# Samleo8/RadarSLAMPy

Hardware: AMD Instinct MI355X
Metric: radar scan-pairs/sec (400x3768 polar) (higher is better)
Workload: dtype u8/f32/f64

## Files before the change

include/roam_abi.h:

```cpp
#ifndef ROAM_ABI_H
#define ROAM_ABI_H
#include <stdint.h>

#ifdef __cplusplus
extern "C" {
#endif

typedef struct roam_ctx roam_ctx;

enum {
    ROAM_OK = 0,
    ROAM_E_ARG = -1,
    ROAM_E_HIP = -2,
    ROAM_E_CAPACITY = -3,
    ROAM_E_NODEVICE = -4,
    ROAM_E_STATE = -5
};

#define ROAM_MAX_FEATURES 1024
#define ROAM_MAX_COLS 4096
#define ROAM_PYR_LEVELS 4

int32_t roam_create(int32_t device_id, roam_ctx **out);
int32_t roam_destroy(roam_ctx *ctx);
// ... 30 lines not shown
                               float *cart_f32, uint8_t *cart_u8);
int32_t roam_polar_to_cart_record_u8(roam_ctx *ctx, const uint8_t *rec, int32_t rows, int64_t stride,
                                     int32_t payload_off, int32_t clip, float *cart_f32,
                                     uint8_t *cart_u8);

#define ROAM_WARP_POLAR_LOG     1
#define ROAM_WARP_POLAR_INVERSE 2
int32_t roam_warp_polar_f32(roam_ctx *ctx, const float *src, int32_t n, int32_t rows, int32_t cols, int64_t src_row_stride,
                            int64_t src_image_stride, float *dst, int32_t dw, int32_t dh, float cx, float cy,
                            double max_radius, int32_t flags);

int32_t roam_klt_track_u8(roam_ctx *ctx, const uint8_t *prev_img, const uint8_t *next_img,
                          int32_t w, int32_t h, const float *pts, int32_t K,
                          float *next_pts, uint8_t *status, float *err);
int32_t roam_klt_track_f32(roam_ctx *ctx, const float *prev_img, const float *next_img,
                           int32_t w, int32_t h, const float *pts, int32_t K,
                           float *next_pts, uint8_t *status, float *err);
int32_t roam_pyr_down_u8(roam_ctx *ctx, const uint8_t *src, int32_t w, int32_t h, uint8_t *dst);

int32_t roam_reject_outliers(roam_ctx *ctx, const float *prev, const float *next, int32_t K,
                             double thr_px, int64_t node_limit, uint8_t *mask_out,
                             int32_t *n_inliers, int32_t *flags_out, uint64_t *adj_out);

int32_t roam_time_reject_outliers(roam_ctx *ctx, const float *prev, const float *next, int32_t K, int32_t copies,
                                  double thr_px, int64_t node_limit, int32_t reps, float *graph_ms, float *clique_ms,
                                  int32_t *n_inliers, int32_t *proven);

int32_t roam_kabsch2d(roam_ctx *ctx, const double *src, const double *tgt, int32_t N,
                      double *R, double *h);

int32_t roam_mds_solve(roam_ctx *ctx, const double *T_wj0, const double *p_w, const double *p_jt,
                       int32_t N, const double *T_wj_init, const double *sigma5, double period,
                       double *out6, int32_t *nfev, int32_t *info, double *x0_out, double *r0_out);
int32_t roam_mds_undistort(roam_ctx *ctx, const double *v3, const double *pts, int32_t N,
                           double period, double *out_xy, double *dT_out);

int32_t roam_ssc(roam_ctx *ctx, const double *kp, int32_t B, int32_t num_ret, double tol,
                 int32_t cols, int32_t rows, int32_t *sel_out, int32_t *n_sel);

int32_t roam_doh_maxima(roam_ctx *ctx, const float *img, int32_t w, int32_t h, const double *sigmas,
                        int32_t num_sigma, double threshold, int32_t *out_rcs, double *out_val,
                        int32_t cap, int32_t *n_out);

int32_t roam_log_maxima(roam_ctx *ctx, const void *img, int32_t img_bytes_per_px, int32_t w, int32_t h, int32_t num_sigma,
                        const int32_t *radius, const double *kernels, const double *scale, double threshold, int32_t *out_rcs,
                        double *out_val, int32_t cap, int32_t *n_out, double *out_layers);

int32_t roam_prune_blobs(const double *blobs, int32_t n, double overlap, uint8_t *keep_out);
int32_t roam_argsort_np122(const double *keys, int32_t n, int32_t *order_out);

int32_t roam_fmt_rotation(roam_ctx *ctx, const float *src_polar, const float *tgt_polar, int32_t rows, int32_t cols,
                          int32_t clip_px, int32_t downsample, double *angle_rad, double *scale, double *response);

int32_t roam_phase_correlate_f32(roam_ctx *ctx, const float *src, const float *tgt, int32_t batch, int32_t rows, int32_t cols,
                                 int64_t row_stride, int64_t image_stride, int32_t hanning, double *out_dxdy, double *out_response);

typedef struct roam_engine_cfg {
    int32_t lanes;
    int32_t rows;
    int32_t stride;
    int32_t payload_off;
    int32_t clip;
    int32_t pool_scans;
    int32_t peaks_cap;
    int32_t reject_outliers;
    int32_t motion_distortion;
// ... 105 lines not shown
```

radarslampy_amd/_ffi.py:

```python
import ctypes as C
import os
import threading

import numpy as np

_HERE = os.path.dirname(os.path.abspath(__file__))
LIB_PATH = os.environ.get("ROAM_LIB") or os.path.join(_HERE, "csrc", "libroam_hip.so")

ROAM_OK, ROAM_E_ARG, ROAM_E_HIP, ROAM_E_CAPACITY, ROAM_E_NODEVICE, ROAM_E_STATE = 0, -1, -2, -3, -4, -5
WARP_POLAR_LOG, WARP_POLAR_INVERSE = 1, 2
TIME_FFT_FIVE, TIME_DFT_FIVE, TIME_FFT_ROWS, TIME_FFT_TRANSPOSE, TIME_FFT_COLS = range(5)
PHASE_CORRELATE_MAX = 4096
MAX_FEATURES = 1024
STEP_NEW_SEQUENCE = 0x40000000


class RoamError(RuntimeError):
    def __init__(self, code, msg):
        super().__init__(f"libroam_hip error {code}: {msg}")
        self.code = code


class EngineCfg(C.Structure):
    _fields_ = [("lanes", C.c_int32), ("rows", C.c_int32), ("stride", C.c_int32), ("payload_off", C.c_int32),
# ... 21 lines not shown
_SIGS = {
    "roam_create": (C.c_int32, [C.c_int32, _P(_vp)]),
    "roam_destroy": (C.c_int32, [_vp]),
    "roam_last_error": (C.c_char_p, [_vp]),
    "roam_version": (C.c_char_p, []),
    "roam_device_info": (C.c_int32, [_vp, C.c_char_p, C.c_int32, _P(C.c_int32), _P(C.c_int64), C.c_char_p, C.c_int32]),
    "roam_synchronize": (C.c_int32, [_vp]),
    "roam_host_alloc": (C.c_int32, [_vp, C.c_int64, _P(_vp)]),
    "roam_host_free": (C.c_int32, [_vp, _vp]),
    "roam_png_decode_gray8": (C.c_int32, [_vp, C.c_int64, _vp, C.c_int64, C.c_int64, _P(C.c_int32), _P(C.c_int32)]),
    "roam_png_decode_file": (C.c_int32, [C.c_char_p, _vp, C.c_int64, C.c_int64, _P(C.c_int32), _P(C.c_int32)]),
    "roam_png_pool_create": (C.c_int32, [C.c_int32, _P(_vp)]),
    "roam_png_pool_submit": (C.c_int32, [_vp, C.c_char_p, _vp, C.c_int64, C.c_int64, C.c_int64]),
    "roam_png_pool_wait": (C.c_int32, [_vp, C.c_int64, _P(C.c_int32), _P(C.c_int32)]),
    "roam_png_pool_destroy": (C.c_int32, [_vp]),
    "roam_peaks_polar_f32": (C.c_int32, [_vp, _vp, C.c_int32, C.c_int32, _vp, C.c_int64, _P(C.c_int64)]),
    "roam_peaks_record_u8": (C.c_int32, [_vp, _vp, C.c_int32, C.c_int64, C.c_int32, C.c_int32, _vp, C.c_int64, _P(C.c_int64)]),
    "roam_peaks_polar_f32_cond": (C.c_int32, [_vp, _vp, C.c_int32, C.c_int32, C.c_double, C.c_double, C.c_double, _vp, C.c_int64,
                                              _P(C.c_int64)]),
    "roam_peaks_record_u8_cond": (C.c_int32, [_vp, _vp, C.c_int32, C.c_int64, C.c_int32, C.c_int32, C.c_double, C.c_double, C.c_double,
                                              _vp, C.c_int64, _P(C.c_int64)]),
    "roam_polar_to_cart_f32": (C.c_int32, [_vp, _vp, C.c_int32, C.c_int32, _vp, _vp]),
    "roam_polar_to_cart_record_u8": (C.c_int32, [_vp, _vp, C.c_int32, C.c_int64, C.c_int32, C.c_int32, _vp, _vp]),
    "roam_warp_polar_f32": (C.c_int32, [_vp, _vp, C.c_int32, C.c_int32, C.c_int32, C.c_int64, C.c_int64, _vp, C.c_int32, C.c_int32,
                                        C.c_float, C.c_float, C.c_double, C.c_int32]),
    "roam_klt_track_u8": (C.c_int32, [_vp, _vp, _vp, C.c_int32, C.c_int32, _vp, C.c_int32, _vp, _vp, _vp]),
    "roam_klt_track_f32": (C.c_int32, [_vp, _vp, _vp, C.c_int32, C.c_int32, _vp, C.c_int32, _vp, _vp, _vp]),
    "roam_pyr_down_u8": (C.c_int32, [_vp, _vp, C.c_int32, C.c_int32, _vp]),
    "roam_reject_outliers": (C.c_int32, [_vp, _vp, _vp, C.c_int32, C.c_double, C.c_int64, _vp, _P(C.c_int32), _P(C.c_int32), _vp]),
    "roam_time_reject_outliers": (C.c_int32, [_vp, _vp, _vp, C.c_int32, C.c_int32, C.c_double, C.c_int64, C.c_int32, _P(C.c_float), _P(C.c_float),
                                               _P(C.c_int32), _P(C.c_int32)]),
    "roam_kabsch2d": (C.c_int32, [_vp, _vp, _vp, C.c_int32, _vp, _vp]),
    "roam_mds_solve": (C.c_int32, [_vp, _vp, _vp, _vp, C.c_int32, _vp, _vp, C.c_double, _vp, _P(C.c_int32), _P(C.c_int32), _vp, _vp]),
    "roam_mds_undistort": (C.c_int32, [_vp, _vp, _vp, C.c_int32, C.c_double, _vp, _vp]),
    "roam_ssc": (C.c_int32, [_vp, _vp, C.c_int32, C.c_int32, C.c_double, C.c_int32, C.c_int32, _vp, _P(C.c_int32)]),
    "roam_doh_maxima": (C.c_int32, [_vp, _vp, C.c_int32, C.c_int32, _vp, C.c_int32, C.c_double, _vp, _vp, C.c_int32, _P(C.c_int32)]),
    "roam_log_maxima": (C.c_int32, [_vp, _vp, C.c_int32, C.c_int32, C.c_int32, C.c_int32, _vp, _vp, _vp, C.c_double, _vp, _vp, C.c_int32,
                                    _P(C.c_int32), _vp]),
    "roam_engine_create": (C.c_int32, [_vp, _P(EngineCfg)]),
    "roam_engine_destroy": (C.c_int32, [_vp]),
    "roam_engine_upload_scan": (C.c_int32, [_vp, C.c_int32, _vp]),
    "roam_engine_upload_scans_async": (C.c_int32, [_vp, C.c_int32, C.c_int32, _vp, C.c_int64]),
    "roam_engine_fence": (C.c_int32, [_vp]),
    "roam_engine_copy_scan": (C.c_int32, [_vp, C.c_int32, C.c_int32]),
    "roam_engine_init_lane": (C.c_int32, [_vp, C.c_int32, C.c_int32, _vp, C.c_int32, _vp]),
    "roam_engine_step": (C.c_int32, [_vp, _vp]),
    "roam_engine_results": (C.c_int32, [_vp, _P(LaneResult), C.c_int32]),
    "roam_engine_step_results": (C.c_int32, [_vp, C.c_int64, _P(LaneResult), C.c_int32]),
    "roam_engine_steps_enqueued": (C.c_int32, [_vp, _P(C.c_int64)]),
    "roam_engine_set_retrack": (C.c_int32, [_vp, C.c_int32]),
    "roam_engine_init_lane_detect": (C.c_int32, [_vp, C.c_int32, C.c_int32, _vp]),
    "roam_engine_init_lanes_detect": (C.c_int32, [_vp, C.c_int32, C.c_int32, _vp, _vp]),
    "roam_engine_lane_features": (C.c_int32, [_vp, C.c_int32, _vp, C.c_int32, _P(C.c_int32)]),
    "roam_engine_lane_peaks": (C.c_int32, [_vp, C.c_int32, _vp, C.c_int64, _P(C.c_int64)]),
    "roam_engine_doh_maxima": (C.c_int32, [_vp, C.c_int32, _vp, C.c_int32, C.c_double, _vp, _vp, C.c_int32, _P(C.c_int32)]),
    "roam_engine_lane_image": (C.c_int32, [_vp, C.c_int32, C.c_int32, _vp, C.c_int64]),
    "roam_engine_set_features": (C.c_int32, [_vp, C.c_int32, _vp, C.c_int32]),
    "roam_engine_kernel_avg": (C.c_int32, [_vp, C.c_char_p, C.c_int32, _P(C.c_float), _P(C.c_int32)]),
    "roam_engine_kernel_chunk_ms": (C.c_int32, [_vp, C.c_char_p, C.c_int32, _P(C.c_float), C.c_int32, _P(C.c_int32), _P(C.c_int32)]),
    "roam_engine_detect_chunk": (C.c_int32, [_vp, _P(C.c_int32)]),
    "roam_engine_map_reserve": (C.c_int32, [_vp, C.c_int32]),
    "roam_engine_map_count": (C.c_int32, [_vp, C.c_int32, _P(C.c_int32)]),
    "roam_engine_map_get": (C.c_int32, [_vp, C.c_int32, C.c_int32, _vp, _vp, _vp, C.c_int32, _P(C.c_int32), _P(C.c_int32)]),
    "roam_engine_stage_times": (C.c_int32, [_vp, _vp, _P(C.c_char_p), C.c_int32, _P(C.c_int32)]),
    "roam_engine_set_stage_events": (C.c_int32, [_vp, C.c_int32]),
    "roam_engine_time_kernel": (C.c_int32, [_vp, C.c_char_p, C.c_int32, _P(C.c_float), _P(C.c_double)]),
# ... 228 lines not shown
        return mask.astype(bool), n_in.value, flags.value, adj

    def time_reject_outliers(self, prev, new, thr_px, copies=4096, reps=3, node_limit=0):
        p = np.ascontiguousarray(prev, np.float32).reshape(-1, 2)
        n = np.ascontiguousarray(new, np.float32).reshape(-1, 2)
        g, q, ni, pr = C.c_float(0), C.c_float(0), C.c_int32(0), C.c_int32(0)
        self.check(self.lib.roam_time_reject_outliers(self.h, _ptr(p), _ptr(n), p.shape[0], int(copies), float(thr_px), int(node_limit), int(reps),
                                                      C.byref(g), C.byref(q), C.byref(ni), C.byref(pr)))
        return float(g.value), float(q.value), ni.value, bool(pr.value)

    def kabsch2d(self, src, tgt):
        s = np.ascontiguousarray(src, np.float64).reshape(-1, 2)
        t = np.ascontiguousarray(tgt, np.float64).reshape(-1, 2)
        R = np.empty((2, 2), np.float64)
        h = np.empty((2, 1), np.float64)
        self.check(self.lib.roam_kabsch2d(self.h, _ptr(s), _ptr(t), s.shape[0], _ptr(R), _ptr(h)))
        return R, h

    def mds_solve(self, T_wj0, p_w, p_jt, T_init, sigma5, period=0.25, want_debug=False):
        T0 = np.ascontiguousarray(T_wj0, np.float64)
        Ti = np.ascontiguousarray(T_init, np.float64)
        pw = np.ascontiguousarray(p_w[:, :2], np.float64)
        pj = np.ascontiguousarray(p_jt[:, :2], np.float64)
        sg = np.ascontiguousarray(sigma5, np.float64)
        N = pw.shape[0]
        out = np.empty(6)
        nfev, info = C.c_int32(0), C.c_int32(0)
        x0 = np.empty(6) if want_debug else None
        r0 = np.empty(2 * N + 3) if want_debug else None
        self.check(self.lib.roam_mds_solve(self.h, _ptr(T0), _ptr(pw), _ptr(pj), N, _ptr(Ti), _ptr(sg), float(period),
                                           _ptr(out), C.byref(nfev), C.byref(info), _ptr(x0), _ptr(r0)))
        return out, nfev.value, info.value, x0, r0

    def mds_undistort(self, v, pts, period=0.25):
        v = np.ascontiguousarray(v, np.float64)
        p = np.ascontiguousarray(pts[:, :2], np.float64)
        N = p.shape[0]
        xy = np.empty((N, 2))
        dT = np.empty(N)
        self.check(self.lib.roam_mds_undistort(self.h, _ptr(v), _ptr(p), N, float(period), _ptr(xy), _ptr(dT)))
        return xy, dT

    def ssc(self, kp, num_ret, tol, cols, rows):
        kp = np.ascontiguousarray(kp, np.float64)
        B = kp.shape[0]
        sel = np.empty(max(B, 1), np.int32)
        n = C.c_int32(0)
        self.check(self.lib.roam_ssc(self.h, _ptr(kp), B, int(num_ret), float(tol), int(cols), int(rows), _ptr(sel), C.byref(n)))
        return sel[:n.value]

    def fmt_rotation(self, src_polar, tgt_polar, clip_px=1012, downsample=10):
        a = np.ascontiguousarray(src_polar, np.float32)
        b = np.ascontiguousarray(tgt_polar, np.float32)
        assert a.shape == b.shape, "Images need to have the same shape!"
        ang, sc, rs = C.c_double(0), C.c_double(0), C.c_double(0)
        self.check(self.lib.roam_fmt_rotation(self.h, _ptr(a), _ptr(b), a.shape[0], a.shape[1], int(clip_px), int(downsample),
                                              C.byref(ang), C.byref(sc), C.byref(rs)))
        return ang.value, sc.value, rs.value

    def phase_correlate(self, src, tgt, hanning=True):
        a, b = phase_correlate_args(src, tgt)
        a, b = _f32_rows_in_place(a), _f32_rows_in_place(b)
        batch = a.ndim == 3
        a3, b3 = (a, b) if batch else (a[None], b[None])
        n, rows, cols = a3.shape
        if a3.strides[0 if n > 1 else 1:] != b3.strides[0 if n > 1 else 1:]:
# ... 74 lines not shown
```

radarslampy_amd/csrc/api.hip:

```cpp
#include "roam_internal.h"
#include <cmath>
#include <cstdlib>
#include <new>

extern "C" {

const char *roam_version(void) { return "radarslampy_amd 0.1 (gfx950, HIP)"; }

int32_t roam_create(int32_t device_id, roam_ctx **out)
{
    if (!out) return ROAM_E_ARG;
    *out = nullptr;
    int ndev = 0;
    if (hipGetDeviceCount(&ndev) != hipSuccess || ndev <= 0) return ROAM_E_NODEVICE;
    if (device_id < 0 || device_id >= ndev) return ROAM_E_ARG;
    roam_ctx *ctx = new (std::nothrow) roam_ctx();
    if (!ctx) return ROAM_E_HIP;
    ctx->device = device_id;
    if (hipSetDevice(device_id) != hipSuccess) { delete ctx; return ROAM_E_HIP; }
    hipDeviceProp_t prop;
    if (hipGetDeviceProperties(&prop, device_id) != hipSuccess) { delete ctx; return ROAM_E_HIP; }
    ctx->cu_count = prop.multiProcessorCount;
    if (hipStreamCreateWithFlags(&ctx->stream, hipStreamNonBlocking) != hipSuccess) { delete ctx; return ROAM_E_HIP; }
    if (hipStreamCreateWithFlags(&ctx->stream2, hipStreamNonBlocking) != hipSuccess) { hipStreamDestroy(ctx->stream); delete ctx; return ROAM_E_HIP; }
// ... 400 lines not shown
    ARG_CHECK(ctx, T_wj0 && p_w && p_jt && T_wj_init && sigma5 && out6 && N >= 2 && N <= 8 * ROAM_MAX_FEATURES && period > 0);
    const size_t m = 2 * (size_t)N + 3;
    SCRATCH(dT, double, S_IN0, sizeof(double) * 18);
    SCRATCH(dpw, double, S_IN1, sizeof(double) * 2 * (size_t)N);
    SCRATCH(dpj, double, S_IN2, sizeof(double) * 2 * (size_t)N);
    SCRATCH(dwork, double, S_TMP0, sizeof(double) * (m * 9 + N));
    SCRATCH(dout, double, S_OUT0, sizeof(double) * (6 + 6));
    SCRATCH(dr0, double, S_OUT1, sizeof(double) * m);
    SCRATCH(dint, int32_t, S_OUT2, sizeof(int32_t) * 2);
    double Tb[18];
    memcpy(Tb, T_wj0, sizeof(double) * 9);
    memcpy(Tb + 9, T_wj_init, sizeof(double) * 9);
    H2D(dT, Tb, sizeof(Tb));
    H2D(dpw, p_w, sizeof(double) * 2 * (size_t)N);
    H2D(dpj, p_jt, sizeof(double) * 2 * (size_t)N);
    MdsProblemDesc P;
    P.T_wj0 = dT; P.T_init = dT + 9; P.p_w = dpw; P.p_jt = dpj; P.count = nullptr;
    P.N = N; P.nstride = N; P.nmax = N; P.B = 1; P.period = period;
    for (int i = 0; i < 5; i++) P.sigma5[i] = sigma5[i];
    HIP_TRY(ctx, launch_mds_solve(ctx->stream, P, dwork, dout, dint, dint + 1, dout + 6, dr0));
    double o[12];
    int32_t ii[2];
    D2H(o, dout, sizeof(o));
    D2H(ii, dint, sizeof(ii));
    if (r0_out) D2H(r0_out, dr0, sizeof(double) * m);
    SYNC();
    memcpy(out6, o, sizeof(double) * 6);
    if (x0_out) memcpy(x0_out, o + 6, sizeof(double) * 6);
    if (nfev) *nfev = ii[0];
    if (info) *info = ii[1];
    return ROAM_OK;
}

extern "C" int32_t roam_mds_undistort(roam_ctx *ctx, const double *v3, const double *pts, int32_t N,
                                      double period, double *out_xy, double *dT_out)
{
    ENTER();
    ARG_CHECK(ctx, v3 && pts && N >= 0 && (out_xy || dT_out));
    if (N == 0) return ROAM_OK;
    SCRATCH(dv, double, S_IN0, sizeof(double) * 3);
    SCRATCH(dp, double, S_IN1, sizeof(double) * 2 * (size_t)N);
    SCRATCH(dxy, double, S_OUT0, sizeof(double) * 2 * (size_t)N);
    SCRATCH(ddt, double, S_OUT1, sizeof(double) * (size_t)N);
    H2D(dv, v3, sizeof(double) * 3);
    H2D(dp, pts, sizeof(double) * 2 * (size_t)N);
    HIP_TRY(ctx, launch_mds_undistort(ctx->stream, dv, dp, N, period, dxy, ddt));
    if (out_xy) D2H(out_xy, dxy, sizeof(double) * 2 * (size_t)N);
    if (dT_out) D2H(dT_out, ddt, sizeof(double) * (size_t)N);
    SYNC();
    return ROAM_OK;
}
```

radarslampy_amd/csrc/engine.hip:

```cpp
#include "roam_internal.h"
#include "retrack.h"
#include "kabsch_body.inc"
#include <algorithm>
#include <new>

#define KS ROAM_MAX_FEATURES
#define CART_CENTER 1012.0
#define M_PER_PX 0.0864
#define N_RETRACK 60
#define ROT_THR 0.2
#define TRANS_THR_SQ 4.0
#define ERR_THR 10.0f
#define TWO_PI 6.283185307179586476925286766559

#define RES_RING 8
enum { ST_PEAKS = 0, ST_WARP, ST_PYR, ST_KLT, ST_GRAPH, ST_CLIQUE, ST_KABSCH, ST_LM, ST_GLUE, ST_RETRACK, ST_COUNT };
static const char *kStageNames[ST_COUNT] = {"ingest_peaks", "warp_quantise", "pyramid", "klt", "consistency_graph",
                                            "max_clique", "kabsch", "mds_lm", "glue", "retrack"};

struct Engine {
    roam_engine_cfg cfg;
    int B = 0, W = 0, stage_cap = 0;
    PyrDesc pd;
    size_t rec_bytes = 0;
// ... 575 lines not shown
    ok = ok && dalloc(ctx, e, &e->feat, (size_t)B * KS * 2);
    ok = ok && dalloc(ctx, e, &e->feat_n, (size_t)B);
    ok = ok && dalloc(ctx, e, &e->klt_next, (size_t)B * KS * 2);
    ok = ok && dalloc(ctx, e, &e->klt_err, (size_t)B * KS);
    ok = ok && dalloc(ctx, e, &e->klt_status, (size_t)B * KS);
    ok = ok && dalloc(ctx, e, &e->good_old, (size_t)B * KS * 2);
    ok = ok && dalloc(ctx, e, &e->good_new, (size_t)B * KS * 2);
    ok = ok && dalloc(ctx, e, &e->good_idx, (size_t)B * KS);
    ok = ok && dalloc(ctx, e, &e->good_n, (size_t)B);
    ok = ok && dalloc(ctx, e, &e->adj, (size_t)B * KS * nw);
    ok = ok && dalloc(ctx, e, &e->cq_stack, (size_t)B * (KS + 2) * 2 * nw);
    ok = ok && dalloc(ctx, e, &e->cq_order, (size_t)B);
    ok = ok && dalloc(ctx, e, &e->cq_mask, (size_t)B * KS);
    ok = ok && dalloc(ctx, e, &e->cq_n, (size_t)B);
    ok = ok && dalloc(ctx, e, &e->cq_flags, (size_t)B);
    ok = ok && dalloc(ctx, e, &e->kab_src, (size_t)B * KS * 2);
    ok = ok && dalloc(ctx, e, &e->kab_tgt, (size_t)B * KS * 2);
    ok = ok && dalloc(ctx, e, &e->kab_out, (size_t)B * 6);
    ok = ok && dalloc(ctx, e, &e->in_n, (size_t)B);
    ok = ok && dalloc(ctx, e, &e->kf_pose, (size_t)B * 3);
    ok = ok && dalloc(ctx, e, &e->kf_vel, (size_t)B * 3) && dalloc(ctx, e, &e->kf_scan, (size_t)B) && dalloc(ctx, e, &e->kf_fresh, (size_t)B) &&
         dalloc(ctx, e, &e->kf_live, (size_t)B) && dalloc(ctx, e, &e->map_n, (size_t)B);
    ok = ok && dalloc(ctx, e, &e->kf_und, (size_t)B * KS * 2);
    ok = ok && dalloc(ctx, e, &e->kf_und_tmp, (size_t)B * KS * 2);
    ok = ok && dalloc(ctx, e, &e->pose, (size_t)B * 3);
    ok = ok && dalloc(ctx, e, &e->vel, (size_t)B * 3);
    ok = ok && dalloc(ctx, e, &e->T_wj0, (size_t)B * 9);
    ok = ok && dalloc(ctx, e, &e->T_init, (size_t)B * 9);
    ok = ok && dalloc(ctx, e, &e->p_w, (size_t)B * KS * 2);
    ok = ok && dalloc(ctx, e, &e->p_jt, (size_t)B * KS * 2);
    ok = ok && dalloc(ctx, e, &e->lm_work, (size_t)B * ((size_t)(2 * KS + 3) * 9 + KS));
    ok = ok && dalloc(ctx, e, &e->lm_out, (size_t)B * 6);
    ok = ok && dalloc(ctx, e, &e->lm_nfev, (size_t)B);
    ok = ok && dalloc(ctx, e, &e->lm_big, (size_t)2 * (1 + B));
    ok = ok && dalloc(ctx, e, &e->lm_info, (size_t)B);
    ok = ok && dalloc(ctx, e, &e->results, (size_t)B * RES_RING);
    if (ok && hipHostMalloc(reinterpret_cast<void **>(&e->results_host), sizeof(roam_lane_result) * (size_t)B * RES_RING, hipHostMallocDefault) != hipSuccess) {
        ROAM_SET_ERR(ctx, "engine: hipHostMalloc failed"); ok = false;
    }
    { const char *se = getenv("ROAM_STAGE_EVENTS"); e->stage_ev = !(se && se[0] == '0'); e->stage_ev_forced = se && (se[0] == '0' || se[0] == '1'); }
    e->rt_on = cfg->retrack_on_device != 0;
    if (ok && e->rt_on) {
        RtArgs &r = e->rt;
        memset(&r, 0, sizeof(r));
        const double step = (10.0 - 0.01) / 2.0;
        r.sigma1 = 1.0 * step + 0.01; r.sigma2 = 10.0; r.threshold = 0.0005;
        r.size1 = (int)(3 * r.sigma1); r.size2 = (int)(3 * r.sigma2);
        r.W = e->W; r.rows = cfg->rows; r.cols = cfg->clip; r.stride = cfg->stride; r.payload_off = cfg->payload_off;
        r.rec_bytes = (int64_t)e->rec_bytes;
        const int R = r.slots = std::max(1, std::min(B, cfg->retrack_slots > 0 ? cfg->retrack_slots : 2048));
        const size_t npx = (size_t)e->W * e->W;
        if (e->W > 2048) { ROAM_SET_ERR(ctx, "engine: device retrack needs a Cartesian image of at most 2048 x 2048"); roam_engine_destroy(ctx); return ROAM_E_ARG; }
        ok = ok && dalloc(ctx, e, &r.rt_n, 2) && dalloc(ctx, e, &r.rt_lane, (size_t)B) && dalloc(ctx, e, &r.rt_scan, (size_t)B);
        r.SP = (e->W + 15) & ~15;
        ok = ok && dalloc(ctx, e, &r.S, (size_t)r.SP * e->W * R);
        ok = ok && dalloc(ctx, e, const_cast<uint32_t **>(&r.boxtab), retrack_boxtab_words(e->W));
        ok = ok && dalloc(ctx, e, const_cast<uint32_t **>(&r.darktab), retrack_darktab_words(e->W));
        ok = ok && dalloc(ctx, e, const_cast<uint32_t **>(&r.phlist), retrack_phase_words(e->W));
        ok = ok && dalloc(ctx, e, &r.colT, (size_t)std::min(R, RT_TWO_PASS_SLOTS) * ((e->W + 63) / 64) * e->W);
        ok = ok && dalloc(ctx, e, &r.col_done, (size_t)std::min(R, RT_TWO_PASS_SLOTS) * 64);
        {
            const char *fv = getenv("ROAM_FUSED_DETECT");
            r.fused = (fv && fv[0] == '1') ? 1 : 0;
            e->det_side.chunk = getenv("ROAM_DET_SIDE") ? atoi(getenv("ROAM_DET_SIDE")) : ((B >= 2048 && r.slots >= 2048) ? 1024 : 0);
            r.fd_halo_words = (int64_t)retrack_fused_halo_words(e->W);
        }
        const size_t D = (size_t)B;
// ... 930 lines not shown
```

radarslampy_amd/csrc/kabsch_mds.hip:

```cpp
#include "roam_internal.h"

#define EPSMCH 2.220446049250313e-16
#define DWARF 2.2250738585072014e-308
#define LM_TMAX 256
#define TWO_PI 6.283185307179586476925286766559

#include "kabsch_body.inc"

__global__ __launch_bounds__(256) void kabsch_kernel(const double *__restrict__ src, const double *__restrict__ tgt,
                                                     const int32_t *__restrict__ count, int N, int nstride,
                                                     double *__restrict__ out6)
{
    __shared__ double red[8];
    const int b = blockIdx.x;
    kabsch_body(src + (int64_t)b * nstride * 2, tgt + (int64_t)b * nstride * 2, count ? count[b] : N, red, out6 + (int64_t)b * 6);
}

hipError_t launch_kabsch(hipStream_t st, const double *src, const double *tgt, const int32_t *count,
                         int N, int nstride, int B, double *out6)
{
    if (B <= 0) return hipSuccess;
    hipLaunchKernelGGL(kabsch_kernel, dim3(B), dim3(256), 0, st, src, tgt, count, N, nstride, out6);
    return hipGetLastError();
}
// ... 499 lines not shown
                    if (S.gnorm <= EPSMCH) info = 8;
                }
                S.info = info;
                S.ratio = ratio;
            }
            __syncthreads();
            if (S.accept) for (int i = t; i < m; i += (int)blockDim.x) fvec[i] = wa4[i];
            const int info = S.info;
            const double ratio = S.ratio;
            __syncthreads();
            LM_TICK(5)
            if (info != 0 || !(ratio < 1e-4)) break;
        }
        if (S.info != 0) break;
    }
#ifdef LM_TIMING
    if (x0_out && t == 0) for (int k = 0; k < 6; k++) x0_out[(size_t)b * 6 + k] = (double)tk[k];
#endif
    if (t < 6) out6[(size_t)b * 6 + t] = S.x[t];
    if (t == 0) { nfev_out[b] = S.nfev; info_out[b] = S.info; }
}

__global__ __launch_bounds__(LM_TMAX, LM_WPE) void mds_lm_kernel(MdsProblemDesc P, double *__restrict__ work_g,
                                                      double *__restrict__ out6, int32_t *__restrict__ nfev_out,
                                                      int32_t *__restrict__ info_out, double *__restrict__ x0_out,
                                                      double *__restrict__ r0_out, int lds_bytes, int wave_rows)
{
    extern __shared__ __align__(16) unsigned char lm_smem[];
    __shared__ LmShared S;
    if (!P.big || wave_rows == 0) {
        mds_lm_block_solve(P, blockIdx.x, work_g, out6, nfev_out, info_out, x0_out, r0_out, lds_bytes, wave_rows, lm_smem, S);
        return;
    }
    const int32_t *L = P.big + (size_t)P.big_slot * (1 + P.B);
    const int nbig = L[0];
    for (int q = blockIdx.x; q < nbig; q += (int)gridDim.x) {
        mds_lm_block_solve(P, L[1 + q], work_g, out6, nfev_out, info_out, x0_out, r0_out, lds_bytes, wave_rows, lm_smem, S);
        __syncthreads();
    }
    if (blockIdx.x == 0 && threadIdx.x == 0) P.big[(size_t)(P.big_slot ^ 1) * (1 + P.B)] = 0;
}

hipError_t launch_mds_solve(hipStream_t st, const MdsProblemDesc &p, double *work, double *out6,
                            int32_t *nfev, int32_t *info, double *x0_out, double *r0_out)
{
    if (p.B <= 0) return hipSuccess;
    const int ppt = std::min(4, (p.nmax + 2 + 63) / 64);
    const int wave_rows = 64 * ppt;
#define LMW_LAUNCH(PPT_) hipLaunchKernelGGL((mds_lm_wave_kernel<PPT_>), dim3(p.B), dim3(64), 0, st, p, out6, nfev, info, x0_out, r0_out)
    switch (ppt) {
    case 1: LMW_LAUNCH(1); break;
    case 2: LMW_LAUNCH(2); break;
    case 3: LMW_LAUNCH(3); break;
    default: LMW_LAUNCH(4); break;
    }
#undef LMW_LAUNCH
    hipError_t e = hipGetLastError();
    if (e != hipSuccess || p.nmax + 2 <= wave_rows) return e;
    const size_t mmax = 2 * (size_t)p.nmax + 3;
    size_t need = (mmax * 9 + p.nmax) * sizeof(double);
    const size_t cap = 32768;
    size_t lds = need <= cap ? need : cap;
    const int threads = p.nmax <= 448 ? 128 : LM_TMAX;
    const int grid = p.big ? std::min(p.B, 512) : p.B;
    hipLaunchKernelGGL(mds_lm_kernel, dim3(grid), dim3(threads), lds, st, p, work, out6, nfev, info, x0_out, r0_out, (int)lds, wave_rows);
    return hipGetLastError();
}

__global__ __launch_bounds__(256) void mds_undistort_kernel(const double *__restrict__ v3, const double *__restrict__ pts,
                                                            int N, double period, double *__restrict__ out_xy,
                                                            double *__restrict__ dT_out)
{
    const int i = blockIdx.x * 256 + threadIdx.x;
    if (i >= N) return;
    const double x = pts[2 * i], y = pts[2 * i + 1];
    const double dT = period * atan2(-y, -x) / TWO_PI;
    const double a = v3[2] * dT, ca = cos(a), sa = sin(a);
    if (out_xy) {
        out_xy[2 * i] = ca * x - sa * y + v3[0] * dT;
        out_xy[2 * i + 1] = sa * x + ca * y + v3[1] * dT;
    }
    if (dT_out) dT_out[i] = dT;
}

hipError_t launch_mds_undistort(hipStream_t st, const double *v3, const double *pts, int N,
                                double period, double *out_xy, double *dT)
{
    if (N <= 0) return hipSuccess;
    hipLaunchKernelGGL(mds_undistort_kernel, dim3((N + 255) / 256), dim3(256), 0, st, v3, pts, N, period, out_xy, dT);
    return hipGetLastError();
// ... 2 lines not shown
```

radarslampy_amd/csrc/lm_wave.inc:

```

struct LmU { double I[6], ip0, ip1, iv0, iv1, iv2, period, Nn; };

__device__ __forceinline__ void lmw_vel_resid(const LmU &U, const double (&x)[6], double ct, double st, double (&out3)[3])
{
    const double tx = x[3], ty = x[4];
    const double m00 = U.I[0] * ct + U.I[1] * st, m10 = U.I[3] * ct + U.I[4] * st;
    const double mdx = U.I[0] * tx + U.I[1] * ty + U.I[2], mdy = U.I[3] * tx + U.I[4] * ty + U.I[5];
    const double dth = atan2(m10, m00);
    const double d0 = x[0] - mdx / U.period, d1 = x[1] - mdy / U.period;
    const double d2 = wrap_pi(x[2] - dth / U.period);
    out3[0] = U.iv0 * (d0 * U.Nn);
    out3[1] = U.iv1 * (d1 * U.Nn);
    out3[2] = U.iv2 * (d2 * U.Nn);
}

__device__ __forceinline__ double lmw_enorm6(const double (&v)[6])
{
    double s = 0;
#pragma unroll
    for (int i = 0; i < 6; i++) s += v[i] * v[i];
    return sqrt(s);
}

__device__ __forceinline__ double lmw_sel6(const double (&v)[6], int idx)
// ... 133 lines not shown
    if (paru == 0) paru = DWARF / (delta < 0.1 ? delta : 0.1);
    if (par < parl) par = parl;
    if (par > paru) par = paru;
    if (par == 0) par = gnorm / dxnorm;
    for (;;) {
        iter++;
        if (par == 0) { const double tq = 0.001 * paru; par = DWARF > tq ? DWARF : tq; }
        double temp = sqrt(par);
        lmw_qrsolv(R, Tl, ipvt, temp, qtb, x, sdiag);
#pragma unroll
        for (int j = 0; j < 6; j++) wa2[j] = x[j];
        dxnorm = lmw_enorm6(wa2);
        temp = fp;
        fp = dxnorm - delta;
        if (fabs(fp) <= 0.1 * delta || (parl == 0 && fp <= temp && temp < 0) || iter == 10) break;
#pragma unroll
        for (int j = 0; j < 6; j++) wa1[j] = lmw_sel6(wa2, ipvt[j]) / dxnorm;
#pragma unroll
        for (int j = 0; j < 6; j++) {
            wa1[j] /= sdiag[j];
            const double tq = wa1[j];
#pragma unroll
            for (int i = j + 1; i < 6; i++) wa1[i] -= Tl[i][j] * tq;
        }
        temp = lmw_enorm6(wa1);
        const double parc = ((fp / delta) / temp) / temp;
        if (fp > 0 && par > parl) parl = par;
        if (fp < 0 && par < paru) paru = par;
        const double np_ = par + parc;
        par = parl > np_ ? parl : np_;
    }
}

template <int PPT>
__global__ __launch_bounds__(64, 2) void mds_lm_wave_kernel(MdsProblemDesc P, double *__restrict__ out6, int32_t *__restrict__ nfev_out,
                                                         int32_t *__restrict__ info_out, double *__restrict__ x0_out,
                                                         double *__restrict__ r0_out)
{
    __shared__ double pts[5][64 * PPT];
    const int b = blockIdx.x, t = threadIdx.x;
    const int N = P.count ? min(P.count[b], P.nmax) : P.N;
    if (N + 2 > 64 * PPT) {
        if (P.big && t == 0) {
            int32_t *L = P.big + (size_t)P.big_slot * (1 + P.B);
            L[1 + atomicAdd(L, 1)] = b;
        }
        return;
    }
    if (N < 2) {
        if (t == 0) { nfev_out[b] = 0; info_out[b] = -1; for (int j = 0; j < 6; j++) out6[(size_t)b * 6 + j] = 0.0; }
        return;
    }
    const int mmax = 2 * P.nmax + 3;
    const double *p_w = P.p_w + (size_t)b * P.nstride * 2;
    const double *p_jt = P.p_jt + (size_t)b * P.nstride * 2;
    const double *T0 = P.T_wj0 + (size_t)b * 9, *Ti = P.T_init + (size_t)b * 9;
    LmU U;
    double x[6];
    {
        const double ta = T0[0], tb = T0[1], tx = T0[2], tc = T0[3], td = T0[4], ty = T0[5];
        const double det = ta * td - tb * tc;
        U.I[0] = td / det; U.I[1] = -tb / det; U.I[3] = -tc / det; U.I[4] = ta / det;
        U.I[2] = -(U.I[0] * tx + U.I[1] * ty); U.I[5] = -(U.I[3] * tx + U.I[4] * ty);
        U.ip0 = 1 / P.sigma5[0]; U.ip1 = 1 / P.sigma5[1];
        U.iv0 = 1 / P.sigma5[2]; U.iv1 = 1 / P.sigma5[3]; U.iv2 = 1 / P.sigma5[4];
        U.period = P.period; U.Nn = (double)N;
        const double r00 = U.I[0] * Ti[0] + U.I[1] * Ti[3], r10 = U.I[3] * Ti[0] + U.I[4] * Ti[3];
        x[0] = (U.I[0] * Ti[2] + U.I[1] * Ti[5] + U.I[2]) / P.period;
        x[1] = (U.I[3] * Ti[2] + U.I[4] * Ti[5] + U.I[5]) / P.period;
        x[2] = atan2(r10, r00) / P.period;
        x[3] = Ti[2]; x[4] = Ti[5]; x[5] = atan2(Ti[3], Ti[0]);
    }
#pragma unroll
    for (int p = 0; p < PPT; p++) {
        const int i = t + 64 * p;
        double px = 0, py = 0, wx = 0, wy = 0, d = 0;
        if (i < N) {
            px = p_jt[2 * i]; py = p_jt[2 * i + 1]; wx = p_w[2 * i]; wy = p_w[2 * i + 1];
            d = P.period * atan2(-py, -px) / TWO_PI;
        }
        pts[0][p * 64 + t] = px; pts[1][p * 64 + t] = py; pts[2][p * 64 + t] = wx; pts[3][p * 64 + t] = wy; pts[4][p * 64 + t] = d;
    }
    if (x0_out && t < 6) {
#pragma unroll
// ... 336 lines not shown
            }
            if (ratio >= 1e-4) {
#pragma unroll
                for (int j = 0; j < 6; j++) x[j] = xtry[j];
                xnorm = lmw_enorm6(x);
                fnorm = fnorm1;
                iter++;
#pragma unroll
                for (int p = 0; p < PPT; p++) { fvec[p][0] = w4[p][0]; fvec[p][1] = w4[p][1]; }
#pragma unroll
                for (int k = 0; k < 3; k++) fvel[k] = v3[k];
            }
            info = 0;
            if (fabs(actred) <= 1e-8 && prered <= 1e-8 && 0.5 * ratio <= 1) info = 1;
            if (delta <= 1e-8 * xnorm) info = 2;
            if (fabs(actred) <= 1e-8 && prered <= 1e-8 && 0.5 * ratio <= 1 && info == 2) info = 3;
            if (info == 0) {
                if (nfev >= 100 * 6 * 7) info = 5;
                if (fabs(actred) <= EPSMCH && prered <= EPSMCH && 0.5 * ratio <= 1) info = 6;
                if (delta <= EPSMCH * xnorm) info = 7;
                if (gnorm <= EPSMCH) info = 8;
            }
            LMW_TICK(5)
            if (info != 0 || !(ratio < 1e-4)) break;
        }
        if (info != 0) break;
    }
#ifdef LM_TIMING
    if (x0_out && t == 0) for (int k = 0; k < 6; k++) x0_out[(size_t)b * 6 + k] = (double)tk[k];
#endif
#pragma unroll
    for (int j = 0; j < 6; j++) if (t == j) out6[(size_t)b * 6 + j] = x[j];
    if (t == 0) { nfev_out[b] = nfev; info_out[b] = info; }
}
```

Baseline: 54070.

## Add mid-tier single-wave LM kernel for 257-382 point problems before block fallback

Adds a second wave-level Levenberg-Marquardt pass with six points per thread (one wave per SIMD) that handles problems too large for the 256-row wave kernel. It works through a device-side todo list, so these problems no longer drop straight to the slower block-level solver. A second pair of big-list slots is introduced and the list-reset logic moves into the new kernel, with the big buffer doubled in size. It also adds a batched host API and profiling scripts. The cost is an extra kernel launch and a larger LDS/register footprint for the mid-tier kernel.

```diff
diff --git a/include/roam_abi.h b/include/roam_abi.h
--- a/include/roam_abi.h
+++ b/include/roam_abi.h
@@ -86,6 +86,9 @@
 int32_t roam_mds_solve(roam_ctx *ctx, const double *T_wj0, const double *p_w, const double *p_jt,
                        int32_t N, const double *T_wj_init, const double *sigma5, double period,
                        double *out6, int32_t *nfev, int32_t *info, double *x0_out, double *r0_out);
+int32_t roam_mds_solve_batch(roam_ctx *ctx, int32_t B, const int32_t *counts, int32_t nstride, int32_t nmax, const double *T_wj0,
+                             const double *p_w, const double *p_jt, const double *T_wj_init, const double *sigma5,
+                             double period, double *out6, int32_t *nfev, int32_t *info);
 int32_t roam_mds_undistort(roam_ctx *ctx, const double *v3, const double *pts, int32_t N,
                            double period, double *out_xy, double *dT_out);
 
diff --git a/profiles/lm_tail_compare.py b/profiles/lm_tail_compare.py
--- /dev/null
+++ b/profiles/lm_tail_compare.py
@@ -0,0 +1,23 @@
+#!/usr/bin/env python3
+import os, sys
+import numpy as np
+a, b = sys.argv[1], sys.argv[2]
+names = sorted(f[:-4] for f in os.listdir(a) if f.endswith(".npy"))
+bad = 0
+for k in names:
+    x, y = np.load(os.path.join(a, k + ".npy")), np.load(os.path.join(b, k + ".npy"))
+    if x.shape != y.shape:
+        print(f"{k:24s} shapes differ {x.shape} {y.shape}"); bad += 1
+        continue
+    ndiff = int(np.count_nonzero(x != y))
+    print(f"{k:24s} {str(x.shape):14s} differing entries {ndiff:6d}   max |diff| {float(np.abs(x - y).max()) if x.size else 0.0:.3e}")
+    if k in ("n_tracked", "n_inliers", "flags") and ndiff:
+        bad += 1
+if "n_inliers" in names and "pose" in names:
+    n = np.load(os.path.join(a, "n_inliers.npy"))
+    d = np.abs(np.load(os.path.join(a, "pose.npy")) - np.load(os.path.join(b, "pose.npy")))
+    for lo, hi in ((0, 254), (255, 10 ** 6)):
+        m = (n >= lo) & (n <= hi)
+        print(f"lanes whose last problem had {lo}..{hi} points: {int(m.sum()):5d}, max pose diff x/y {float(d[m][:, :2].max()) if m.any() else 0.0:.3e} m, theta {float(d[m][:, 2].max()) if m.any() else 0.0:.3e} rad")
+print("counts and flags equal" if not bad else f"{bad} count / flag columns DIFFER")
+sys.exit(1 if bad else 0)
diff --git a/profiles/lm_tail_lone.py b/profiles/lm_tail_lone.py
--- /dev/null
+++ b/profiles/lm_tail_lone.py
@@ -0,0 +1,29 @@
+#!/usr/bin/env python3
+import os, sys
+ROOT = os.path.dirname(os.path.dirname(os.path.abspath(__file__)))
+SIZES, REPS = (255, 300, 350, 382), 10
+if len(sys.argv) > 2 and sys.argv[1] == "--parse":
+    import csv, glob, statistics
+    f = sorted(glob.glob(sys.argv[2] + "/*/*kernel_trace.csv"))[0]
+    rows = sorted((int(r["Start_Timestamp"]), int(r["End_Timestamp"]) - int(r["Start_Timestamp"]), r["Kernel_Name"].split("(")[0]) for r in csv.DictReader(open(f)))
+    work = [(d, n) for _, d, n in rows if "mds_lm" in n and d > 40000]
+    assert len(work) == len(SIZES) * REPS, len(work)
+    for i, N in enumerate(SIZES):
+        seg = work[i * REPS:(i + 1) * REPS]
+        print(f"N {N:4d}  {seg[0][1]:40s} median {statistics.median(d for d, _ in seg) / 1e3:8.1f} us  min {min(d for d, _ in seg) / 1e3:8.1f}  max {max(d for d, _ in seg) / 1e3:8.1f}")
+    sys.exit(0)
+sys.path.insert(0, ROOT)
+sys.path.insert(0, os.path.join(ROOT, "tests", "golden"))
+import numpy as np
+from gen_inputs import mds_problem
+from radarslampy_amd import _ffi
+if len(sys.argv) > 2 and sys.argv[1] == "--lib":
+    _ffi.LIB_PATH = os.path.abspath(sys.argv[2])
+ctx = _ffi.Context(0)
+sigma5 = np.array([4, 4, 1, 1, (5 * np.pi / 180) ** 2], np.float64)
+for N in SIZES:
+    T0, p_w, p_jt, Tinit, _ = mds_problem(N, 100 + N, 0.05)
+    for rep in range(REPS):
+        out = ctx.mds_solve(T0, p_w, p_jt, Tinit, sigma5)
+    print("N", N, "nfev", out[1], "info", out[2])
+ctx.close()
diff --git a/profiles/lm_tail_sizes.py b/profiles/lm_tail_sizes.py
--- /dev/null
+++ b/profiles/lm_tail_sizes.py
@@ -0,0 +1,66 @@
+#!/usr/bin/env python3
+import argparse, json, os, sys
+import numpy as np
+ROOT = os.path.dirname(os.path.dirname(os.path.abspath(__file__)))
+sys.path.insert(0, ROOT)
+ap = argparse.ArgumentParser()
+ap.add_argument("--lanes", type=int, default=4096)
+ap.add_argument("--steps", type=int, default=20)
+ap.add_argument("--warmup", type=int, default=5)
+ap.add_argument("--preroll", type=int, default=16)
+ap.add_argument("--lib", default=None)
+a = ap.parse_args()
+import bench
+from radarslampy_amd import _ffi
+if a.lib:
+    _ffi.LIB_PATH = os.path.abspath(a.lib)
+from radarslampy_amd.engine import Engine
+
+B, T, Dn = a.lanes, 7, min(16, a.lanes)
+seqs = bench.render_sequences([17 * d + 5 for d in range(Dn)], T, True, bench.WORK_RETRACK, 0)
+ctx = _ffi.Context(0)
+en = Engine(B, B * T, ctx=ctx, motion_distortion=True, retrack_on_device=True)
+for d in range(Dn):
+    for t in range(T):
+        en.upload_scan(d * T + t, seqs[d][0][t])
+for b in range(Dn, B):
+    for t in range(T):
+        en.copy_scan(b * T + t, (b % Dn) * T + t)
+en.synchronize()
+period = 2 * T - 2
+cyc = np.array(list(range(T)) + list(range(T - 2, 0, -1)))
+phase = np.array([(b // Dn) % period for b in range(B)])
+t0s = cyc[phase]
+en.init_lanes_detect(0, [b * T + t0s[b] for b in range(B)], np.array([seqs[b % Dn][1][t0s[b]] for b in range(B)]))
+
+
+def step(i):
+    ph = (phase + i + 1) % period
+    en.step(((np.arange(B) * T + cyc[ph]) | np.where(ph == 0, _ffi.STEP_NEW_SEQUENCE, 0)).astype(np.int32))
+
+
+s = 0
+for _ in range(a.preroll + a.warmup):
+    step(s); s += 1
+first = s
+sizes = []
+for k in range(a.steps):
+    step(s); s += 1
+    if (k + 1) % 8 == 0 or k == a.steps - 1:
+        en.synchronize()
+        for q in range(first + len(sizes), s):
+            r = en.results_array(q)
+            sizes.append(r["n_inliers"].astype(np.int64))
+sizes = np.array(sizes)
+edges = [0, 2, 64, 128, 192, 255, 319, 383, 447, 511, 1025]
+hist = np.histogram(sizes, bins=edges)[0]
+out = {"lanes": B, "steps": int(sizes.shape[0]), "problems": int(sizes.size), "max_points": int(sizes.max()),
+       "mean_points": round(float(sizes.mean()), 1),
+       "histogram": {f"{lo}..{hi - 1}": int(n) for lo, hi, n in zip(edges[:-1], edges[1:], hist)}}
+for lim in (254, 318, 382, 446, 510):
+    per = (sizes > lim).sum(axis=1)
+    out[f"per_step_above_{lim}"] = {"min": int(per.min()), "mean": round(float(per.mean()), 1), "max": int(per.max())}
+out["largest_per_step"] = [int(v) for v in sizes.max(axis=1)]
+print(json.dumps(out))
+en.close()
+ctx.close()
diff --git a/profiles/lm_tail_trace.py b/profiles/lm_tail_trace.py
--- /dev/null
+++ b/profiles/lm_tail_trace.py
@@ -0,0 +1,39 @@
+#!/usr/bin/env python3
+import csv, glob, re, sys
+f = sorted(glob.glob(sys.argv[1] + "/*/*kernel_trace.csv"))[0]
+K = int(sys.argv[2]) if len(sys.argv) > 2 else 20
+rows = [(int(r["Start_Timestamp"]), int(r["End_Timestamp"]), r["Kernel_Name"]) for r in csv.DictReader(open(f))]
+rows.sort()
+
+
+def short(n):
+    m = re.search(r"(mds_lm_wave_kernel<[^>]*>|mds_lm_kernel|g2_inliers_kernel|rt_integral_kernel)", n)
+    return m.group(1).replace(" ", "") if m else None
+
+
+ev = [(s, e, short(n)) for s, e, n in rows if short(n)]
+g2 = [i for i, x in enumerate(ev) if x[2] == "g2_inliers_kernel"]
+g2 = g2[-K:]
+names, table = [], []
+for n, i in enumerate(g2):
+    hi = g2[n + 1] if n + 1 < len(g2) else len(ev)
+    seg = ev[i:hi]
+    d = {}
+    for s, e, k in seg[1:]:
+        if k.startswith("mds_lm"):
+            d[k] = d.get(k, 0.0) + (e - s) / 1e6
+            if k not in names:
+                names.append(k)
+    lm = [x for x in seg if x[2].startswith("mds_lm")]
+    rt = [x for x in seg if x[2] == "rt_integral_kernel" and lm and x[0] >= lm[0][0]]
+    small = [x for x in lm if x[2].startswith("mds_lm_wave_kernel")][:1]
+    d["gap"] = (rt[0][0] - seg[0][1]) / 1e6 if rt else float("nan")
+    d["tail"] = (rt[0][0] - small[0][1]) / 1e6 if rt and small else float("nan")
+    table.append(d)
+cols = sorted(names) + ["gap", "tail"]
+print("step " + " ".join(f"{c[-24:]:>24s}" for c in cols) + "     (ms; gap = g2_inliers end -> first rt_integral start; tail = first wave kernel end -> first rt_integral start)")
+for n, d in enumerate(table):
+    print(f"{n:4d} " + " ".join(f"{d.get(c, 0.0):24.3f}" for c in cols))
+ok = [d for d in table if d["gap"] == d["gap"]]
+for tag, fn in (("mean", lambda v: sum(v) / len(v)), ("min", min), ("max", max)):
+    print(f"{tag:>4s} " + " ".join(f"{fn([d.get(c, 0.0) for d in ok]):24.3f}" for c in cols))
diff --git a/radarslampy_amd/_ffi.py b/radarslampy_amd/_ffi.py
--- a/radarslampy_amd/_ffi.py
+++ b/radarslampy_amd/_ffi.py
@@ -77,6 +77,7 @@
                                                _P(C.c_int32), _P(C.c_int32)]),
     "roam_kabsch2d": (C.c_int32, [_vp, _vp, _vp, C.c_int32, _vp, _vp]),
     "roam_mds_solve": (C.c_int32, [_vp, _vp, _vp, _vp, C.c_int32, _vp, _vp, C.c_double, _vp, _P(C.c_int32), _P(C.c_int32), _vp, _vp]),
+    "roam_mds_solve_batch": (C.c_int32, [_vp, C.c_int32, _vp, C.c_int32, C.c_int32, _vp, _vp, _vp, _vp, _vp, C.c_double, _vp, _vp, _vp]),
     "roam_mds_undistort": (C.c_int32, [_vp, _vp, _vp, C.c_int32, C.c_double, _vp, _vp]),
     "roam_ssc": (C.c_int32, [_vp, _vp, C.c_int32, C.c_int32, C.c_double, C.c_int32, C.c_int32, _vp, _P(C.c_int32)]),
     "roam_doh_maxima": (C.c_int32, [_vp, _vp, C.c_int32, C.c_int32, _vp, C.c_int32, C.c_double, _vp, _vp, C.c_int32, _P(C.c_int32)]),
@@ -371,6 +372,22 @@
                                            _ptr(out), C.byref(nfev), C.byref(info), _ptr(x0), _ptr(r0)))
         return out, nfev.value, info.value, x0, r0
 
+    def mds_solve_batch(self, problems, sigma5, period=0.25, nmax=0):
+        B = len(problems)
+        cnt = np.array([len(p[1]) for p in problems], np.int32)
+        ns = max(1, int(cnt.max()), int(nmax))
+        T0 = np.ascontiguousarray([p[0] for p in problems], np.float64).reshape(B, 9)
+        Ti = np.ascontiguousarray([p[3] for p in problems], np.float64).reshape(B, 9)
+        pw, pj = np.zeros((B, ns, 2)), np.zeros((B, ns, 2))
+        for b, p in enumerate(problems):
+            pw[b, :cnt[b]] = np.asarray(p[1], np.float64)[:, :2]
+            pj[b, :cnt[b]] = np.asarray(p[2], np.float64)[:, :2]
+        sg = np.ascontiguousarray(sigma5, np.float64)
+        out, nfev, info = np.empty((B, 6)), np.empty(B, np.int32), np.empty(B, np.int32)
+        self.check(self.lib.roam_mds_solve_batch(self.h, B, _ptr(cnt), ns, int(nmax), _ptr(T0), _ptr(pw), _ptr(pj), _ptr(Ti), _ptr(sg), float(period),
+                                                 _ptr(out), _ptr(nfev), _ptr(info)))
+        return out, nfev, info
+
     def mds_undistort(self, v, pts, period=0.25):
         v = np.ascontiguousarray(v, np.float64)
         p = np.ascontiguousarray(pts[:, :2], np.float64)
diff --git a/radarslampy_amd/csrc/api.hip b/radarslampy_amd/csrc/api.hip
--- a/radarslampy_amd/csrc/api.hip
+++ b/radarslampy_amd/csrc/api.hip
@@ -456,6 +456,48 @@
     return ROAM_OK;
 }
 
+extern "C" int32_t roam_mds_solve_batch(roam_ctx *ctx, int32_t B, const int32_t *counts, int32_t nstride, int32_t nmax_in, const double *T_wj0,
+                                        const double *p_w, const double *p_jt, const double *T_wj_init, const double *sigma5,
+                                        double period, double *out6, int32_t *nfev, int32_t *info)
+{
+    ENTER();
+    ARG_CHECK(ctx, B >= 1 && B <= 65536 && counts && nstride >= 1 && nstride <= 8 * ROAM_MAX_FEATURES && T_wj0 && p_w && p_jt && T_wj_init &&
+                   sigma5 && out6 && nfev && info && period > 0 && nmax_in >= 0 && nmax_in <= nstride);
+    int nmax = 0;
+    for (int b = 0; b < B; b++) {
+        ARG_CHECK(ctx, counts[b] >= 0 && counts[b] <= nstride);
+        nmax = counts[b] > nmax ? counts[b] : nmax;
+    }
+    ARG_CHECK(ctx, nmax_in == 0 || nmax_in >= nmax);
+    nmax = nmax_in ? nmax_in : (nmax < 1 ? 1 : nmax);
+    const size_t npt = (size_t)B * nstride * 2, m = 2 * (size_t)nmax + 3;
+    SCRATCH(dT, double, S_IN0, sizeof(double) * 18 * (size_t)B);
+    SCRATCH(dpw, double, S_IN1, sizeof(double) * npt);
+    SCRATCH(dpj, double, S_IN2, sizeof(double) * npt);
+    SCRATCH(dcnt, int32_t, S_IN3, sizeof(int32_t) * (size_t)B);
+    SCRATCH(dwork, double, S_TMP0, sizeof(double) * (m * 9 + nmax) * (size_t)B);
+    SCRATCH(dbig, int32_t, S_TMP1, sizeof(int32_t) * 4 * (1 + (size_t)B));
+    SCRATCH(dout, double, S_OUT0, sizeof(double) * 6 * (size_t)B);
+    SCRATCH(dint, int32_t, S_OUT2, sizeof(int32_t) * 2 * (size_t)B);
+    H2D(dT, T_wj0, sizeof(double) * 9 * (size_t)B);
+    H2D(dT + 9 * (size_t)B, T_wj_init, sizeof(double) * 9 * (size_t)B);
+    H2D(dpw, p_w, sizeof(double) * npt);
+    H2D(dpj, p_jt, sizeof(double) * npt);
+    H2D(dcnt, counts, sizeof(int32_t) * (size_t)B);
+    HIP_TRY(ctx, hipMemsetAsync(dbig, 0, sizeof(int32_t) * 4 * (1 + (size_t)B), ctx->stream));
+    MdsProblemDesc P;
+    P.T_wj0 = dT; P.T_init = dT + 9 * (size_t)B; P.p_w = dpw; P.p_jt = dpj; P.count = dcnt;
+    P.N = nmax; P.nstride = nstride; P.nmax = nmax; P.B = B; P.period = period;
+    for (int i = 0; i < 5; i++) P.sigma5[i] = sigma5[i];
+    P.big = dbig; P.big_slot = 0;
+    HIP_TRY(ctx, launch_mds_solve(ctx->stream, P, dwork, dout, dint, dint + B, nullptr, nullptr));
+    D2H(out6, dout, sizeof(double) * 6 * (size_t)B);
+    D2H(nfev, dint, sizeof(int32_t) * (size_t)B);
+    D2H(info, dint + B, sizeof(int32_t) * (size_t)B);
+    SYNC();
+    return ROAM_OK;
+}
+
 extern "C" int32_t roam_mds_undistort(roam_ctx *ctx, const double *v3, const double *pts, int32_t N,
                                       double period, double *out_xy, double *dT_out)
 {
diff --git a/radarslampy_amd/csrc/engine.hip b/radarslampy_amd/csrc/engine.hip
--- a/radarslampy_amd/csrc/engine.hip
+++ b/radarslampy_amd/csrc/engine.hip
@@ -631,7 +631,7 @@
     ok = ok && dalloc(ctx, e, &e->lm_work, (size_t)B * ((size_t)(2 * KS + 3) * 9 + KS));
     ok = ok && dalloc(ctx, e, &e->lm_out, (size_t)B * 6);
     ok = ok && dalloc(ctx, e, &e->lm_nfev, (size_t)B);
-    ok = ok && dalloc(ctx, e, &e->lm_big, (size_t)2 * (1 + B));
+    ok = ok && dalloc(ctx, e, &e->lm_big, (size_t)4 * (1 + B));
     ok = ok && dalloc(ctx, e, &e->lm_info, (size_t)B);
     ok = ok && dalloc(ctx, e, &e->results, (size_t)B * RES_RING);
     if (ok && hipHostMalloc(reinterpret_cast<void **>(&e->results_host), sizeof(roam_lane_result) * (size_t)B * RES_RING, hipHostMallocDefault) != hipSuccess) {
diff --git a/radarslampy_amd/csrc/kabsch_mds.hip b/radarslampy_amd/csrc/kabsch_mds.hip
--- a/radarslampy_amd/csrc/kabsch_mds.hip
+++ b/radarslampy_amd/csrc/kabsch_mds.hip
@@ -555,22 +555,23 @@
         mds_lm_block_solve(P, blockIdx.x, work_g, out6, nfev_out, info_out, x0_out, r0_out, lds_bytes, wave_rows, lm_smem, S);
         return;
     }
-    const int32_t *L = P.big + (size_t)P.big_slot * (1 + P.B);
+    const int32_t *L = P.big + (size_t)(2 + P.big_slot) * (1 + P.B);
     const int nbig = L[0];
     for (int q = blockIdx.x; q < nbig; q += (int)gridDim.x) {
         mds_lm_block_solve(P, L[1 + q], work_g, out6, nfev_out, info_out, x0_out, r0_out, lds_bytes, wave_rows, lm_smem, S);
         __syncthreads();
     }
-    if (blockIdx.x == 0 && threadIdx.x == 0) P.big[(size_t)(P.big_slot ^ 1) * (1 + P.B)] = 0;
-}
+}
+
+#define LMW_BIG 6
 
 hipError_t launch_mds_solve(hipStream_t st, const MdsProblemDesc &p, double *work, double *out6,
                             int32_t *nfev, int32_t *info, double *x0_out, double *r0_out)
 {
     if (p.B <= 0) return hipSuccess;
     const int ppt = std::min(4, (p.nmax + 2 + 63) / 64);
-    const int wave_rows = 64 * ppt;
-#define LMW_LAUNCH(PPT_) hipLaunchKernelGGL((mds_lm_wave_kernel<PPT_>), dim3(p.B), dim3(64), 0, st, p, out6, nfev, info, x0_out, r0_out)
+    int wave_rows = 64 * ppt;
+#define LMW_LAUNCH(PPT_) hipLaunchKernelGGL((mds_lm_wave_kernel<PPT_, 2, 0>), dim3(p.B), dim3(64), 0, st, p, out6, nfev, info, x0_out, r0_out)
     switch (ppt) {
     case 1: LMW_LAUNCH(1); break;
     case 2: LMW_LAUNCH(2); break;
@@ -579,6 +580,11 @@
     }
 #undef LMW_LAUNCH
     hipError_t e = hipGetLastError();
+    if (e != hipSuccess || p.nmax + 2 <= wave_rows) return e;
+    const int grid_big = p.big ? std::min(p.B, 1024) : p.B;
+    hipLaunchKernelGGL((mds_lm_wave_kernel<LMW_BIG, 1, 256>), dim3(grid_big), dim3(64), 0, st, p, out6, nfev, info, x0_out, r0_out);
+    wave_rows = 64 * LMW_BIG;
+    e = hipGetLastError();
     if (e != hipSuccess || p.nmax + 2 <= wave_rows) return e;
     const size_t mmax = 2 * (size_t)p.nmax + 3;
     size_t need = (mmax * 9 + p.nmax) * sizeof(double);
diff --git a/radarslampy_amd/csrc/lm_wave.inc b/radarslampy_amd/csrc/lm_wave.inc
--- a/radarslampy_amd/csrc/lm_wave.inc
+++ b/radarslampy_amd/csrc/lm_wave.inc
@@ -189,24 +189,39 @@
     }
 }
 
-template <int PPT>
-__global__ __launch_bounds__(64, 2) void mds_lm_wave_kernel(MdsProblemDesc P, double *__restrict__ out6, int32_t *__restrict__ nfev_out,
-                                                         int32_t *__restrict__ info_out, double *__restrict__ x0_out,
-                                                         double *__restrict__ r0_out)
+template <int PPT, int WPS, int LO>
+__global__ __launch_bounds__(64, WPS) void mds_lm_wave_kernel(MdsProblemDesc P, double *__restrict__ out6, int32_t *__restrict__ nfev_out,
+                                                           int32_t *__restrict__ info_out, double *__restrict__ x0_out,
+                                                           double *__restrict__ r0_out)
 {
     __shared__ double pts[5][64 * PPT];
-    const int b = blockIdx.x, t = threadIdx.x;
+    const int t = threadIdx.x;
+    const int32_t *todo = nullptr;
+    int ntodo = (int)gridDim.x;
+    if (LO > 0 && P.big) {
+        todo = P.big + (size_t)P.big_slot * (1 + P.B);
+        ntodo = todo[0];
+        if (blockIdx.x == 0 && t == 0) {
+            P.big[(size_t)(P.big_slot ^ 1) * (1 + P.B)] = 0;
+            P.big[(size_t)(2 + (P.big_slot ^ 1)) * (1 + P.B)] = 0;
+        }
+        if ((int)blockIdx.x >= ntodo) return;
+    }
+    int q = blockIdx.x;
+    do {
+    const int b = (LO > 0 && todo) ? todo[1 + q] : q;
     const int N = P.count ? min(P.count[b], P.nmax) : P.N;
+    if (LO > 0 && N + 2 <= LO) continue;
     if (N + 2 > 64 * PPT) {
         if (P.big && t == 0) {
-            int32_t *L = P.big + (size_t)P.big_slot * (1 + P.B);
+            int32_t *L = P.big + (size_t)((LO > 0 ? 2 : 0) + P.big_slot) * (1 + P.B);
             L[1 + atomicAdd(L, 1)] = b;
         }
-        return;
+        continue;
     }
     if (N < 2) {
         if (t == 0) { nfev_out[b] = 0; info_out[b] = -1; for (int j = 0; j < 6; j++) out6[(size_t)b * 6 + j] = 0.0; }
-        return;
+        continue;
     }
     const int mmax = 2 * P.nmax + 3;
     const double *p_w = P.p_w + (size_t)b * P.nstride * 2;
@@ -609,4 +624,5 @@
 #pragma unroll
     for (int j = 0; j < 6; j++) if (t == j) out6[(size_t)b * 6 + j] = x[j];
     if (t == 0) { nfev_out[b] = nfev; info_out[b] = info; }
+    } while (LO > 0 && (q += (int)gridDim.x) < ntodo);
 }
```

Result: slower. 53320 (-1.4%).
